# lukedan/libfluid

Hardware: AMD Instinct MI355X
Metric: particle_steps_per_sec (higher is better)
Workload: dtype f32

## Files before the change

### include/libfluid_amd.h

```cpp
#ifndef LIBFLUID_AMD_H
#define LIBFLUID_AMD_H

#include <stddef.h>
#include <stdint.h>

#ifdef __cplusplus
extern "C" {
#endif

typedef struct lfa_sim lfa_sim;

enum {
	LFA_OK = 0,
	LFA_E_INVALID = -1,
	LFA_E_NO_DEVICE = -2,
	LFA_E_HIP = -3,
	LFA_E_OOM = -4,
	LFA_E_NAN = -5,
	LFA_E_UNSUPPORTED = -6,
	LFA_W_PCG_NOT_CONVERGED = 1
};

enum { LFA_PIC = 0, LFA_FLIP_BLEND = 1, LFA_APIC = 2 };
enum { LFA_P2G_LDS_BINNED = 0, LFA_P2G_GLOBAL_ATOMIC = 1 };
// ... 115 lines not shown
int lfa_mesher_create_window(lfa_mesher **out, const uint64_t size[3], const double grid_offset[3], double cell_size,
                             double particle_extent, uint64_t cell_radius, uint64_t zlo, uint64_t zhi, int device);
int lfa_mesher_window(const lfa_mesher *m, uint64_t *z0, uint64_t *n_planes, uint64_t *own_lo, uint64_t *own_hi);
int lfa_mesher_sample_ids(lfa_mesher *m, const double *positions, const uint32_t *ids, uint64_t n, double r);
int lfa_mesher_rebase(lfa_mesher *m, uint64_t vertices_below);
int lfa_mesher_create(lfa_mesher **out, const uint64_t size[3], const double grid_offset[3], double cell_size,
                      double particle_extent, uint64_t cell_radius, int device);
void lfa_mesher_destroy(lfa_mesher *m);
const char *lfa_mesher_last_error(const lfa_mesher *m);
int lfa_mesher_sample(lfa_mesher *m, const double *positions, uint64_t n, double r);
int lfa_mesher_sample_sim(lfa_mesher *m, lfa_sim *s, double r);
int lfa_mesher_download_values(lfa_mesher *m, double *values);
int lfa_mesher_upload_values(lfa_mesher *m, const double *values);
int lfa_mesher_marching_cubes(lfa_mesher *m, uint64_t *n_vertices, uint64_t *n_indices);
int lfa_mesher_download_mesh(lfa_mesher *m, double *positions, uint64_t *indices);
int lfa_mesher_normals(lfa_mesher *m);
int lfa_mesher_download_normals(lfa_mesher *m, double *normals);
int lfa_mesher_normals_time(lfa_mesher *m, double *ms);
int lfa_mesher_boundary_size(lfa_mesher *m, uint64_t *n_cells, uint64_t *n_triangles);
int lfa_mesher_download_boundary(lfa_mesher *m, uint8_t *cases, double *face);
int lfa_mesher_window_normals(lfa_mesher *m, const uint8_t *cases_above, const double *face_above, uint64_t n_triangles_above);
int lfa_mesher_window_normals_from(lfa_mesher *m, lfa_mesher *above);

#define LFA_NUM_TIMERS 10
int lfa_enable_timing(lfa_sim *s, int on);
int lfa_get_timings(lfa_sim *s, double ms[LFA_NUM_TIMERS]);
int lfa_get_counts(lfa_sim *s, uint64_t counts[5]);
#define LFA_NUM_SOLVER_STATS 8
int lfa_get_solver_stats(lfa_sim *s, uint64_t stats[LFA_NUM_SOLVER_STATS]);
#define LFA_MAX_MG_LEVELS 12
int lfa_get_mg_level_tiles(lfa_sim *s, uint64_t tiles[LFA_MAX_MG_LEVELS]);
int lfa_get_correction_stats(lfa_sim *s, uint64_t stats[2]);
int lfa_get_correction_stats_ex(lfa_sim *s, uint64_t stats[3]);

enum {
	LFA_K_SPMV_DOT = 0,
	LFA_K_AXPY_MAX = 1,
	LFA_K_MIC_APPLY = 2,
	LFA_K_UPDATE_S = 3,
	LFA_K_P2G_SCATTER = 4,
	LFA_K_P2G_FINALIZE = 5,
	LFA_K_G2P = 6,
	LFA_K_BIN = 7,
	LFA_K_MIC_FINE = 8,
	LFA_K_COARSE = 9,
	LFA_K_PCG_A = 10,
	LFA_K_PCG_B = 11,
	LFA_K_MG_AXPY_PRESMOOTH = 12,
	LFA_K_MG_DOWN0 = 13,
	LFA_K_MG_COARSE = 14,
	LFA_K_MG_UP0 = 15
};
int lfa_bench_kernel(lfa_sim *s, int which, int reps, double *mean_ms);
int lfa_bench_stream(lfa_sim *s, uint64_t bytes, int reps, double *copy_gbs, double *read_gbs);
void lfa_pool_trim(void);
void lfa_pool_stats(uint64_t stats[4]);
const char *lfa_bench_stream_variant(void);

#ifdef __cplusplus
}
#endif
#endif
```

### libfluid_amd/__init__.py

```python
import ctypes as C
import os

import numpy as np

from . import scenes
from .scenes import CELL_DTYPE, PARTICLE_DTYPE

HERE = os.path.dirname(os.path.abspath(__file__))
LIB_PATH = os.path.join(HERE, "libfluid_amd.so")

PIC, FLIP_BLEND, APIC = 0, 1, 2
P2G_LDS_BINNED, P2G_GLOBAL_ATOMIC = 0, 1
PRECOND_MIC0_TILED, PRECOND_MIC0_EXACT, PRECOND_MULTILEVEL, PRECOND_MULTIGRID = 0, 1, 2, 3
PCG_F32, PCG_F64 = 0, 1
OK, W_PCG_NOT_CONVERGED = 0, 1
NUM_TIMERS = 10
NUM_STEP_TIMERS = 16
STEP_TIMER_NAMES = ["advect_collide", "bin", "p2g", "p2g_scatter_kernel", "build_system", "pcg_loop", "apply_pressure",
                    "correct_cell_index", "correct_tiled_kernel", "correct_collide", "extrapolate", "g2p", "time_step",
                    "pcg_iterations", "pcg_iteration_mean", "overlapped"]
TIMER_NAMES = ["bin", "p2g", "gravity", "build_system", "pcg_loop", "apply_pressure", "extrapolate", "g2p",
               "p2g_scatter_kernel", "pcg_iteration_mean"]


# ... 95 lines not shown
    "lfa_mesher_create": (_int, [C.POINTER(_vp), _vp, _vp, _dbl, _dbl, _u64, _int]),
    "lfa_mesher_create_window": (_int, [C.POINTER(_vp), _vp, _vp, _dbl, _dbl, _u64, _u64, _u64, _int]),
    "lfa_mesher_window": (_int, [_vp, C.POINTER(_u64), C.POINTER(_u64), C.POINTER(_u64), C.POINTER(_u64)]),
    "lfa_mesher_sample_ids": (_int, [_vp, _vp, _vp, _u64, _dbl]),
    "lfa_mesher_rebase": (_int, [_vp, _u64]),
    "lfa_mesher_destroy": (None, [_vp]),
    "lfa_mesher_last_error": (C.c_char_p, [_vp]),
    "lfa_mesher_sample": (_int, [_vp, _vp, _u64, _dbl]),
    "lfa_mesher_sample_sim": (_int, [_vp, _vp, _dbl]),
    "lfa_mesher_download_values": (_int, [_vp, _vp]),
    "lfa_mesher_upload_values": (_int, [_vp, _vp]),
    "lfa_mesher_marching_cubes": (_int, [_vp, C.POINTER(_u64), C.POINTER(_u64)]),
    "lfa_mesher_download_mesh": (_int, [_vp, _vp, _vp]),
    "lfa_mesher_normals": (_int, [_vp]),
    "lfa_mesher_download_normals": (_int, [_vp, _vp]),
    "lfa_mesher_normals_time": (_int, [_vp, C.POINTER(_dbl)]),
    "lfa_mesher_boundary_size": (_int, [_vp, C.POINTER(_u64), C.POINTER(_u64)]),
    "lfa_mesher_download_boundary": (_int, [_vp, _vp, _vp]),
    "lfa_mesher_window_normals": (_int, [_vp, _vp, _vp, _u64]),
    "lfa_mesher_window_normals_from": (_int, [_vp, _vp]),
    "lfa_clear_sources": (_int, [_vp]),
    "lfa_add_source": (_int, [_vp, _vp, _u64, _vp, _u64, _int, _int]),
    "lfa_update_sources": (_int, [_vp, C.POINTER(_u64)]),
    "lfa_advect_collide": (_int, [_vp, _dbl]),
    "lfa_advect": (_int, [_vp, _dbl]),
    "lfa_correct": (_int, [_vp, _dbl]),
    "lfa_collide": (_int, [_vp]),
    "lfa_correct_collide": (_int, [_vp, _dbl]),
    "lfa_time_step": (_int, [_vp, _dbl, C.POINTER(_dbl), C.POINTER(_u64)]),
    "lfa_get_step_timings": (_int, [_vp, C.POINTER(_dbl * NUM_STEP_TIMERS)]),
    "lfa_set_step_overlap": (_int, [_vp, _int]),
    "lfa_get_correction_stats": (_int, [_vp, C.POINTER(_u64 * 2)]),
    "lfa_get_correction_stats_ex": (_int, [_vp, C.POINTER(_u64 * 3)]),
    "lfa_correct_collide_begin": (_int, [_vp, _dbl]),
    "lfa_correct_collide_end": (_int, [_vp]),
    "lfa_correct_collide_undo": (_int, [_vp]),
    "lfa_dist_unique_id": (_int, [_vp]),
    "lfa_dist_init_rccl": (_int, [_vp, _int, _int, _vp, _vp]),
    "lfa_dist_local_hub_create": (_vp, [_int]),
    "lfa_dist_local_hub_destroy": (None, [_vp]),
    "lfa_dist_init_local": (_int, [_vp, _vp, _int, _vp]),
    "lfa_dist_init_shm": (_int, [_vp, C.c_char_p, _int, _int, _vp]),
    "lfa_dist_get_slab": (_int, [_vp, C.POINTER(C.c_int32), C.POINTER(C.c_int32)]),
    "lfa_dist_abandon": (_int, [_vp]),
}
KERNELS = {"spmv_dot": 0, "axpy_max": 1, "mic_apply_dot": 2, "update_s": 3, "p2g_scatter": 4, "p2g_finalize": 5,
           "g2p": 6, "bin": 7, "mic_fine": 8, "coarse_levels": 9, "pcg_a": 10, "pcg_b": 11,
           "mg_axpy_presmooth": 12, "mg_down0": 13, "mg_coarse": 14, "mg_up0": 15}


def load_library():
    global _lib
    if _lib is None:
        path = os.environ.get("LFA_LIB_PATH") or LIB_PATH
        if not os.path.exists(path):
            raise ImportError(
                f"{path} is missing: build it with `python -c 'import __graft_entry__ as g; g.build()'` "
                "(there is no CPU fallback for the hot path)")
        lib = C.CDLL(path)
        for name, (res, args) in SIGNATURES.items():
            fn = getattr(lib, name)
            fn.restype, fn.argtypes = res, args
        _lib = lib
    return _lib


# ... 488 lines not shown

    def correct_collide(self, dt):
        self._chk(self.lib.lfa_correct_collide(self.h, float(dt)))

    def correct_collide_begin(self, dt):
        self._chk(self.lib.lfa_correct_collide_begin(self.h, float(dt)))

    def correct_collide_end(self):
        self._chk(self.lib.lfa_correct_collide_end(self.h))

    def correct_collide_undo(self):
        self._chk(self.lib.lfa_correct_collide_undo(self.h))

    def time_step(self, dt):
        res, it = C.c_double(0.0), C.c_uint64(0)
        rc = self._chk(self.lib.lfa_time_step(self.h, float(dt), C.byref(res), C.byref(it)))
        return res.value, it.value, rc

    def step_timings(self):
        arr = (C.c_double * NUM_STEP_TIMERS)()
        self._chk(self.lib.lfa_get_step_timings(self.h, C.byref(arr)))
        return dict(zip(STEP_TIMER_NAMES, list(arr)))

    def correction_stats(self):
        arr = (C.c_uint64 * 2)()
        self._chk(self.lib.lfa_get_correction_stats(self.h, C.byref(arr)))
        return int(arr[0]), int(arr[1])

    def correction_stats_ex(self):
        arr = (C.c_uint64 * 3)()
        self._chk(self.lib.lfa_get_correction_stats_ex(self.h, C.byref(arr)))
        return int(arr[0]), int(arr[1]), int(arr[2])

    def set_step_overlap(self, on):
        self._chk(self.lib.lfa_set_step_overlap(self.h, int(bool(on))))

    def init_local_slab(self, hub, rank, layer_bounds):
        b = np.ascontiguousarray(layer_bounds, dtype=np.int32)
        self._chk(self.lib.lfa_dist_init_local(self.h, hub, int(rank), _ptr(b)))

    def init_rccl_slab(self, rank, nranks, unique_id, layer_bounds):
        b = np.ascontiguousarray(layer_bounds, dtype=np.int32)
        uid = np.frombuffer(bytes(unique_id), dtype=np.uint8).copy()
        self._chk(self.lib.lfa_dist_init_rccl(self.h, int(rank), int(nranks), _ptr(uid), _ptr(b)))

    def init_shm_slab(self, name, rank, nranks, layer_bounds):
        b = np.ascontiguousarray(layer_bounds, dtype=np.int32)
        self._chk(self.lib.lfa_dist_init_shm(self.h, str(name).encode(), int(rank), int(nranks), _ptr(b)))

    def abandon_transport(self):
        self._chk(self.lib.lfa_dist_abandon(self.h))

    def slab(self):
        lo, hi = C.c_int32(0), C.c_int32(0)
        self._chk(self.lib.lfa_dist_get_slab(self.h, C.byref(lo), C.byref(hi)))
        return lo.value, hi.value

    def enable_timing(self, on=True):
        self._chk(self.lib.lfa_enable_timing(self.h, 1 if on else 0))

    def timings(self):
        arr = (C.c_double * NUM_TIMERS)()
        self._chk(self.lib.lfa_get_timings(self.h, C.byref(arr)))
        return dict(zip(TIMER_NAMES, list(arr)))

    def bench_kernel(self, name, reps=20):
# ... 29 lines not shown
```

### libfluid_amd/csrc/particles.hip

```cpp
#include <math.h>

#include <algorithm>
#include <utility>

#include "common.h"
#include "pcg.h"

namespace {

__device__ inline bool solid_or_outside(const GridDims &g, const uint8_t *solid, int x, int y, int z) {
	if (!in_grid(g, x, y, z)) return true;
	return solid[blocked_index(g, x, y, z)] != 0;
}

__device__ inline void collide(const GridDims &g, const uint8_t *solid, double from[3], double to[3], double skin) {
	for (int bounce = 0; bounce < 3; ++bounce) {
		bool hit = false;
		double diff[3], inv[3], t[3];
		int cur[3], last[3], adv[3];
#pragma unroll
		for (int d = 0; d < 3; ++d) {
			cur[d] = (int)floor(from[d]);
			last[d] = (int)floor(to[d]);
			diff[d] = to[d] - from[d];
// ... 58 lines not shown
		const double cp = to[d] - (double)ci;
		double x = to[d];
		if (cp < skin && ci == 0) x += skin - cp;
		if (cp > skin_max && ci + 1 >= n[d]) x += skin_max - cp;
		to[d] = x;
	}
}

__device__ inline void cell_of_key(const GridDims &g, uint32_t key, int c[3]) {
	int tile = (int)(key >> 9), l = (int)(key & 511), tx, ty, tz;
	tile_coords(g, tile, tx, ty, tz);
	c[0] = tx * 8 + (l & 7); c[1] = ty * 8 + ((l >> 3) & 7); c[2] = tz * 8 + (l >> 6);
}
__device__ inline void split_position(double p, int n, int &cell, float &t) {
	double m = p < 0.0 ? 0.0 : p;
	int c = m >= (double)n ? n - 1 : (int)m;
	double td = p - (double)c;
	float tf = (float)td;
	if (!(tf > 0.0f)) tf = 0.0f;
	if (td < 1.0 && tf >= 1.0f) tf = 0.99999994f;
	if (tf > 1.0f) tf = 1.0f;
	cell = c;
	t = tf;
}

#ifndef CORR_PARTS
#define CORR_PARTS 2
#endif
#define CORR_THREADS 512
#define CORR_THREADS_BIG 1024
#ifndef CORR_STAGE_DEPTH
#define CORR_STAGE_DEPTH 4
#endif
#define CORR_BIG_SLICES 4

struct MoveParams {
	double dt_over_h;
	double skin;
	double corr;
	double inv_re2;
	float *c_home;
	size_t c_home_stride;
	int collide;
};

__global__ void __launch_bounds__(256) k_tile_has_solid(const uint8_t *solid, int nt, uint8_t *tile_solid) {
	for (int t = blockIdx.x; t < nt; t += gridDim.x) {
		const uint8_t *c = solid + (size_t)t * LFA_TILE_CELLS;
		const int any = __syncthreads_or((c[threadIdx.x] | c[threadIdx.x + 256]) != 0);
		if (threadIdx.x == 0) tile_solid[t] = (uint8_t)(any ? 1 : 0);
	}
}
__global__ void k_tile_clear(GridDims g, const uint8_t *tile_solid, uint8_t *tile_clear) {
	const int t = blockIdx.x * blockDim.x + threadIdx.x;
	if (t >= g.nt) return;
	int tx, ty, tz;
	tile_coords(g, t, tx, ty, tz);
	int any = 0;
	for (int dz = -1; dz <= 1; ++dz)
		for (int dy = -1; dy <= 1; ++dy)
			for (int dx = -1; dx <= 1; ++dx) {
				const int x = tx + dx, y = ty + dy, z = tz + dz;
				if ((unsigned)x < (unsigned)g.ntx && (unsigned)y < (unsigned)g.nty && (unsigned)z < (unsigned)g.ntz)
					any |= tile_solid[x + g.ntx * (y + g.nty * z)];
			}
	tile_clear[t] = (uint8_t)(any ? 0 : 1);
// ... 57 lines not shown
}

#define AC_CHUNKS 8
template <bool COERCE>
__global__ void __launch_bounds__(256)
k_advect_collide_count(size_t n, ParticleSoA p, GridDims g, const uint8_t *solid, MoveParams mp, const uint8_t *coerce_map,
                       const float *src_vel, const uint8_t *tile_clear, uint32_t *tile_count, uint32_t *rank) {
	const int lane = threadIdx.x & 63;
	const size_t wave = ((size_t)blockIdx.x * blockDim.x + threadIdx.x) >> 6;
	const size_t i0 = wave * (64 * AC_CHUNKS) + lane;
	uint32_t tile[AC_CHUNKS], my_rank[AC_CHUNKS];
#pragma unroll
	for (int c = 0; c < AC_CHUNKS; ++c) {
		const size_t i = i0 + 64 * c;
		const uint32_t k = i < n ? advect_one<COERCE>(i, p, g, solid, mp, coerce_map, src_vel, tile_clear) : 0xFFFFFFFFu;
		tile[c] = k != 0xFFFFFFFFu ? k >> 9 : 0xFFFFFFFFu;
	}
	lfa_wave_tile_ranks(tile, tile_count, my_rank);
#pragma unroll
	for (int c = 0; c < AC_CHUNKS; ++c) {
		const size_t i = i0 + 64 * c;
		if (tile[c] != 0xFFFFFFFFu) rank[i] = my_rank[c];
	}
}

__device__ inline float hash_unit(uint32_t a, uint32_t b, uint32_t k) {
	uint32_t x = a * 0x9E3779B1u ^ (b + 0x7F4A7C15u) * 0x85EBCA77u ^ k * 0xC2B2AE3Du;
	x ^= x >> 15; x *= 0x2C1B3C6Du; x ^= x >> 12; x *= 0x297A2D39u; x ^= x >> 15;
	return (float)(x >> 8) * (2.0f / 16777216.0f) - 1.0f;
}

#define FT 11
#define FT3 (FT * FT * FT)
#define FT_STRIDE (FT3 + 1)
#define FT_INV 1.375f
#define FT_PL ((FT + CORR_PARTS - 1) / CORR_PARTS)
#define FB 13
#define FBZ (FT_PL + 2)
#define FB_N (FB * FB * FBZ)
#define FB_ROWS (FB * FBZ)
#define FINE_CAP 5632
#define FINE_CAP_BIG 12288
#define FIDX_THREADS 512
#define FIDX_CNT 1536
#define FIDX_STAGE 4608

__device__ inline int fine_coord(int l, float t) {
	const int f = (int)(((float)l + t) * FT_INV);
	return f < FT - 1 ? f : FT - 1;
}
__device__ inline float4 fine_record(int lx, int ly, int lz, float t0, float t1, float t2, uint32_t index) {
	const uint32_t b0 = (__float_as_uint(t0) & 0x3FFFFFFFu) | ((uint32_t)(lx & 3) << 30);
	const uint32_t b1 = (__float_as_uint(t1) & 0x3FFFFFFFu) | ((uint32_t)(lx >> 2) << 31) | ((uint32_t)(ly & 1) << 30);
	const uint32_t b2 = (__float_as_uint(t2) & 0x3FFFFFFFu) | ((uint32_t)(lz & 1) << 31);
	return make_float4(__uint_as_float(b0), __uint_as_float(b1), __uint_as_float(b2), __uint_as_float(index));
}
__device__ inline void fine_decode(const float4 &r, int fy, int fz, float t[3], int l[3]) {
	const uint32_t b0 = __float_as_uint(r.x), b1 = __float_as_uint(r.y), b2 = __float_as_uint(r.z);
	t[0] = __uint_as_float(b0 & 0x3FFFFFFFu); t[1] = __uint_as_float(b1 & 0x3FFFFFFFu); t[2] = __uint_as_float(b2 & 0x3FFFFFFFu);
	l[0] = (int)(b0 >> 30) | ((int)(b1 >> 31) << 2);
	const int y0 = (8 * fy) / FT, z0 = (8 * fz) / FT;
	l[1] = y0 + ((y0 ^ (int)(b1 >> 30)) & 1);
	l[2] = z0 + ((z0 ^ (int)(b2 >> 31)) & 1);
}

__global__ void __launch_bounds__(FIDX_THREADS)
k_build_fine_index(const int *ptiles, int n_ptiles, const uint32_t *key, const float *t0, const float *t1, const float *t2,
                   const uint32_t *tile_start, const uint32_t *tile_count, uint32_t *fine_start, float4 *spos, uint32_t *key_copy) {
	__shared__ uint32_t cnt[FIDX_CNT];
	__shared__ uint32_t wsum[FIDX_THREADS / 64];
	__shared__ float4 stage[FIDX_STAGE];
	static_assert(FIDX_CNT % FIDX_THREADS == 0 && FIDX_STAGE % FIDX_THREADS == 0, "index kernel sizing");
	constexpr int PER = FIDX_CNT / FIDX_THREADS;
	auto fine_of = [&](uint32_t i, int l[3], float t[3]) -> int {
		const uint32_t k = key[i];
		l[0] = (int)(k & 7); l[1] = (int)((k >> 3) & 7); l[2] = (int)((k >> 6) & 7);
		t[0] = t0[i]; t[1] = t1[i]; t[2] = t2[i];
		return fine_coord(l[0], t[0]) + FT * (fine_coord(l[1], t[1]) + FT * fine_coord(l[2], t[2]));
	};
	constexpr int RPT = FIDX_STAGE / FIDX_THREADS;
	for (int slot = blockIdx.x; slot < n_ptiles; slot += gridDim.x) {
		const int tile = ptiles[slot];
		const uint32_t b = tile_start[tile], e = b + tile_count[tile];
		const bool staged = e - b <= FIDX_STAGE;
#pragma unroll
		for (int k = 0; k < PER; ++k) cnt[threadIdx.x + FIDX_THREADS * k] = 0;
		__syncthreads();
		uint32_t rf[RPT];
		float r0[RPT], r1[RPT], r2[RPT];
		if (staged) {
#pragma unroll
			for (int r = 0; r < RPT; ++r) {
				const uint32_t i = b + threadIdx.x + FIDX_THREADS * r;
				rf[r] = 0xFFFFFFFFu;
				if (i < e) {
					int l[3];
					float t[3];
					const int f = fine_of(i, l, t);
					rf[r] = ((uint32_t)f << 9) | (uint32_t)(l[0] | (l[1] << 3) | (l[2] << 6));
					r0[r] = t[0]; r1[r] = t[1]; r2[r] = t[2];
					atomicAdd(&cnt[f], 1u);
				}
			}
		} else {
			for (uint32_t i = b + threadIdx.x; i < e; i += FIDX_THREADS) {
				int l[3];
				float t[3];
				atomicAdd(&cnt[fine_of(i, l, t)], 1u);
			}
		}
		__syncthreads();
		uint32_t c[PER], incl = 0;
#pragma unroll
		for (int k = 0; k < PER; ++k) {
			c[k] = cnt[PER * threadIdx.x + k];
			incl += c[k];
		}
		const uint32_t sum = incl;
		const int lane = threadIdx.x & 63, wid = threadIdx.x >> 6;
#pragma unroll
		for (int o = 1; o < 64; o <<= 1) {
			uint32_t t = __shfl_up(incl, o, 64);
			if (lane >= o) incl += t;
		}
		if (lane == 63) wsum[wid] = incl;
		__syncthreads();
		uint32_t ex = b + incl - sum;
		for (int w = 0; w < wid; ++w) ex += wsum[w];
		__syncthreads();
#pragma unroll
		for (int k = 0; k < PER; ++k) {
			const int f = PER * threadIdx.x + k;
			cnt[f] = ex;
			if (f <= FT3) fine_start[(size_t)tile * FT_STRIDE + f] = ex;
			ex += c[k];
		}
		__syncthreads();
		if (staged) {
#pragma unroll
			for (int r = 0; r < RPT; ++r)
				if (rf[r] != 0xFFFFFFFFu) {
					const uint32_t at = atomicAdd(&cnt[rf[r] >> 9], 1u);
					stage[at - b] = fine_record((int)(rf[r] & 7), (int)((rf[r] >> 3) & 7), (int)((rf[r] >> 6) & 7), r0[r], r1[r], r2[r],
					                            b + threadIdx.x + FIDX_THREADS * r);
				}
			if (key_copy) {
#pragma unroll
				for (int r = 0; r < RPT; ++r)
					if (rf[r] != 0xFFFFFFFFu) key_copy[b + threadIdx.x + FIDX_THREADS * r] = ((uint32_t)tile << 9) | (rf[r] & 511u);
			}
			__syncthreads();
			for (uint32_t k = threadIdx.x; k < e - b; k += FIDX_THREADS) spos[b + k] = stage[k];
		} else {
			for (uint32_t i = b + threadIdx.x; i < e; i += FIDX_THREADS) {
				int l[3];
				float t[3];
				const uint32_t at = atomicAdd(&cnt[fine_of(i, l, t)], 1u);
				spos[at] = fine_record(l[0], l[1], l[2], t[0], t[1], t[2], i);
				if (key_copy) key_copy[i] = key[i];
			}
		}
		__syncthreads();
	}
}

__device__ inline int fine_source(const GridDims &g, const uint32_t *tile_count, int tx, int ty, int tz, int gx, int gy, int gz, int &fx,
                                  int &fy, int &fz) {
	const int dx = gx < 0 ? -1 : (gx >= FT ? 1 : 0), dy = gy < 0 ? -1 : (gy >= FT ? 1 : 0), dz = gz < 0 ? -1 : (gz >= FT ? 1 : 0);
	fx = gx - FT * dx; fy = gy - FT * dy; fz = gz - FT * dz;
	const int x = tx + dx, y = ty + dy, z = tz + dz;
	if ((unsigned)x >= (unsigned)g.ntx || (unsigned)y >= (unsigned)g.nty || (unsigned)z >= (unsigned)g.ntz) return -1;
	const int tile = x + g.ntx * (y + g.nty * z);
	return tile_count[tile] ? tile : -1;
}

__device__ inline void correct_collide_record(size_t rk, const ParticleSoA &p, uint32_t *out_key, float *out_tx, float *out_ty, float *out_tz,
                                              const GridDims &g, const uint8_t *solid, const uint32_t *tile_count, const uint32_t *fine_start,
                                              const float4 *spos, const MoveParams &mp, const uint32_t *only_flagged, const int *tile_pslot,
                                              int p_off, const uint32_t *key_before) {
	const float4 me = spos[rk];
	const size_t i = __float_as_uint(me.w);
	const uint32_t key_i = key_before ? key_before[i] : p.key[i];
	if (key_i == 0xFFFFFFFFu) return;
	const int tile = (int)(key_i >> 9);
	const int l[3] = {(int)(key_i & 7), (int)((key_i >> 3) & 7), (int)((key_i >> 6) & 7)};
	const float t[3] = {__uint_as_float(__float_as_uint(me.x) & 0x3FFFFFFFu), __uint_as_float(__float_as_uint(me.y) & 0x3FFFFFFFu),
// ... 63 lines not shown
                   const uint8_t *solid, const uint32_t *tile_count, const uint32_t *fine_start, const float4 *spos, MoveParams mp,
                   const uint32_t *only_flagged, const int *tile_pslot, int p_off, const uint32_t *key_before) {
	if (only_flagged && only_flagged[0] == 0) return;
	for (size_t rk = (size_t)blockIdx.x * blockDim.x + threadIdx.x; rk < n; rk += (size_t)gridDim.x * blockDim.x)
		correct_collide_record(rk, p, out_key, out_tx, out_ty, out_tz, g, solid, tile_count, fine_start, spos, mp, only_flagged, tile_pslot,
		                       p_off, key_before);
}

#ifdef CORR_PROFILE
__device__ unsigned long long g_corr_prof[8];
#define CORR_STAMP(k)                                                                   \
	do {                                                                                \
		if (!ONLY && threadIdx.x == 0) {                                                \
			const unsigned long long now_ = wall_clock64();                             \
			atomicAdd(&g_corr_prof[k], now_ - stamp_);                                  \
			stamp_ = now_;                                                              \
		}                                                                               \
	} while (0)
#else
#define CORR_STAMP(k) do { } while (0)
#endif
template <int CAP, bool ONLY>
__global__ void __launch_bounds__(ONLY ? CORR_THREADS_BIG : CORR_THREADS, 4)
k_correct_fine(const int *ptiles, int n_ptiles, uint32_t *out_key, float *out_tx, float *out_ty, float *out_tz, GridDims g,
                const uint8_t *solid, const uint32_t *tile_count, const uint32_t *fine_start, const float4 *spos, MoveParams mp,
                uint32_t *overflow_tiles, const uint8_t *tile_clear, const uint32_t *only) {
	constexpr int T = ONLY ? CORR_THREADS_BIG : CORR_THREADS;
	constexpr int CNT = ((FB_N + 1 + T - 1) / T) * T;
	__shared__ float px[CAP], py[CAP], pz[CAP];
	__shared__ uint32_t fcnt[CNT];
	__shared__ uint16_t foff[FB_N + 1];
	__shared__ uint32_t rowsrc[FB_ROWS * 3];
	__shared__ uint32_t ownoff[FT * FT_PL + 1];
	__shared__ int srct[27];
	__shared__ uint32_t wsum[T / 64];
	uint16_t *own = (uint16_t *)fcnt;
	static_assert(CNT > FB_N && CNT % T == 0, "fcnt sizing");
	constexpr int PER = CNT / T;
	const int nn[3] = {g.nx, g.ny, g.nz};
	const int lane = threadIdx.x & 63, wid = threadIdx.x >> 6;
	if (ONLY && only[0] == 0) return;
	constexpr int SLICES = ONLY ? CORR_BIG_SLICES : 1;
	for (int item = blockIdx.x; item < SLICES * CORR_PARTS * n_ptiles; item += gridDim.x) {
		const int work = item / SLICES, slice = item % SLICES;
		if (ONLY && !((only[1 + (work >> 5)] >> (work & 31)) & 1u)) continue;
		const int tile = ptiles[work / CORR_PARTS], part = work % CORR_PARTS;
		int tx, ty, tz;
		tile_coords(g, tile, tx, ty, tz);
		const int own_lo = part * FT_PL, own_n = (own_lo + FT_PL <= FT ? FT_PL : FT - own_lo);
		const int gz0 = own_lo - 1;
		const int nzb = own_n + 2;
		const int nrows = FB * nzb, nown_rows = FT * (nzb - 2);
		const bool open_water = (tile_clear[tile] & 1) != 0;
		__syncthreads();
#ifdef CORR_PROFILE
		unsigned long long stamp_ = wall_clock64();
		if (!ONLY && threadIdx.x == 0) atomicAdd(&g_corr_prof[7], 1ull);
#endif
		if (threadIdx.x < 27) {
			int fx, fy, fz;
			srct[threadIdx.x] = fine_source(g, tile_count, tx, ty, tz, FT * ((int)threadIdx.x % 3 - 1), FT * (((int)threadIdx.x / 3) % 3 - 1),
			                                FT * ((int)threadIdx.x / 9 - 1), fx, fy, fz);
		}
		__syncthreads();
#pragma unroll
		for (int k = 0; k < PER; ++k) {
			const int f = threadIdx.x + T * k;
			uint32_t cnt = 0, src0 = 0;
			if (f < FB * nrows) {
				const int bx = f % FB, row = f / FB, by = row % FB, bz = row / FB;
				const int gx = bx - 1, gy = by - 1, gz = gz0 + bz;
				const int dx = gx < 0 ? 0 : (gx >= FT ? 2 : 1), dy = gy < 0 ? 0 : (gy >= FT ? 2 : 1), dz = gz < 0 ? 0 : (gz >= FT ? 2 : 1);
				const int src = srct[dx + 3 * dy + 9 * dz];
				if (src >= 0) {
					const uint32_t fid = (uint32_t)((gx - FT * (dx - 1)) + FT * ((gy - FT * (dy - 1)) + FT * (gz - FT * (dz - 1))));
					const uint32_t *fs = fine_start + ((uint32_t)src * FT_STRIDE + fid);
					src0 = fs[0];
					cnt = fs[1] - src0;
				}
				if (bx <= 1 || bx == FB - 1) rowsrc[row * 3 + (bx <= 1 ? bx : 2)] = src0;
			}
			fcnt[f] = cnt;
		}
		__syncthreads();
		uint32_t c4[PER], sum = 0;
#pragma unroll
		for (int k = 0; k < PER; ++k) {
			c4[k] = fcnt[PER * threadIdx.x + k];
			sum += c4[k];
		}
		uint32_t incl = sum;
#pragma unroll
		for (int o = 1; o < 64; o <<= 1) {
			uint32_t t = __shfl_up(incl, o, 64);
			if (lane >= o) incl += t;
		}
		if (lane == 63) wsum[wid] = incl;
// ... 17 lines not shown
				const int f = PER * threadIdx.x + k;
				if (f <= FB_N) foff[f] = (uint16_t)ex;
				ex += c4[k];
			}
		}
		__syncthreads();
		uint32_t own_total = 0;
		{
			uint32_t len = 0;
			if (threadIdx.x < (unsigned)nown_rows) {
				const int row = (1 + threadIdx.x % FT) + FB * (1 + threadIdx.x / FT);
				len = (uint32_t)foff[row * FB + FB - 1] - (uint32_t)foff[row * FB + 1];
			}
			uint32_t in2 = len;
#pragma unroll
			for (int o = 1; o < 64; o <<= 1) {
				uint32_t t = __shfl_up(in2, o, 64);
				if (lane >= o) in2 += t;
			}
			if (lane == 63) wsum[wid] = in2;
			__syncthreads();
			uint32_t wo = 0;
			for (int w = 0; w < T / 64; ++w) {
				if (w < wid) wo += wsum[w];
				own_total += wsum[w];
			}
			if (threadIdx.x < (unsigned)nown_rows) ownoff[threadIdx.x] = wo + in2 - len;
			if (threadIdx.x == 0) ownoff[nown_rows] = own_total;
		}
		const bool listed = own_total <= 2u * CNT;
		__syncthreads();
		CORR_STAMP(0);
		{
			auto locate = [&](uint32_t slot, uint32_t &src, int &seg, int &dy, int &dz, int &fy, int &fz, int &ownslot) {
				int r = 0;
#pragma unroll
				for (int step = 64; step; step >>= 1) {
					const int c = r + step;
					if (c < nrows && (uint32_t)foff[c * FB] <= slot) r = c;
				}
				const int by = r % FB, bz = r / FB;
				const int gy = by - 1, gz = gz0 + bz;
				dy = gy < 0 ? -1 : (gy >= FT ? 1 : 0); dz = gz < 0 ? -1 : (gz >= FT ? 1 : 0);
				fy = gy - FT * dy; fz = gz - FT * dz;
				const uint32_t d0 = foff[r * FB], d1 = foff[r * FB + 1], d2 = foff[r * FB + FB - 1];
				seg = slot < d1 ? 0 : (slot < d2 ? 1 : 2);
				src = rowsrc[r * 3 + seg] + (slot - (seg == 0 ? d0 : (seg == 1 ? d1 : d2)));
				ownslot = (listed && seg == 1 && by >= 1 && by <= FT && bz >= 1 && bz <= nzb - 2)
				              ? (int)(ownoff[(by - 1) + FT * (bz - 1)] + (slot - d1)) : -1;
			};
			auto put = [&](uint32_t slot, const float4 &rec, int seg, int dy, int dz, int fy, int fz, int ownslot) {
				float t[3];
				int l[3];
				fine_decode(rec, fy, fz, t, l);
				px[slot] = (float)(8 * (seg - 1) + l[0]) + t[0];
				py[slot] = (float)(8 * dy + l[1]) + t[1];
				pz[slot] = (float)(8 * dz + l[2]) + t[2];
				if (ownslot >= 0) own[ownslot] = (uint16_t)slot;
			};
			for (uint32_t slot0 = threadIdx.x; slot0 < total; slot0 += CORR_STAGE_DEPTH * T) {
				uint32_t src[CORR_STAGE_DEPTH];
				int meta[CORR_STAGE_DEPTH], ownslot[CORR_STAGE_DEPTH];
				float4 rec[CORR_STAGE_DEPTH];
#pragma unroll
				for (int u = 0; u < CORR_STAGE_DEPTH; ++u) {
					const uint32_t slot = slot0 + u * T;
// ... 13 lines not shown
						put(slot, rec[u], meta[u] & 3, ((meta[u] >> 2) & 3) - 1, ((meta[u] >> 4) & 3) - 1, (meta[u] >> 6) & 15, (meta[u] >> 10) & 15, ownslot[u]);
				}
			}
		}
		__syncthreads();
		CORR_STAMP(1);
#ifdef CORR_PROFILE
		if (!ONLY && threadIdx.x == 0) { atomicAdd(&g_corr_prof[5], (unsigned long long)total); atomicAdd(&g_corr_prof[6], (unsigned long long)own_total); }
#endif
		for (uint32_t w = threadIdx.x + T * slice; w < own_total; w += T * SLICES) {
			uint32_t me;
			if (listed) {
				me = own[w];
			} else {
				int lo = 0, hi = nown_rows - 1;
				while (lo < hi) {
					const int mid = (lo + hi + 1) >> 1;
					if (ownoff[mid] <= w) lo = mid;
					else hi = mid - 1;
				}
				me = (uint32_t)foff[((1 + lo % FT) + FB * (1 + lo / FT)) * FB + 1] + (w - ownoff[lo]);
			}
#ifdef CORR_PROFILE
			const unsigned long long w0_ = wall_clock64();
#endif
			const float mx = px[me], my = py[me], mz = pz[me];
			int fx = (int)(mx * FT_INV), fy = (int)(my * FT_INV), fz = (int)(mz * FT_INV);
			fx = fx < FT - 1 ? fx : FT - 1; fy = fy < FT - 1 ? fy : FT - 1; fz = fz < FT - 1 ? fz : FT - 1;
			const int bx = fx + 1, by = fy + 1, bz = fz - gz0;
			float sx = 0.f, sy = 0.f, sz = 0.f;
			typedef float f2 __attribute__((ext_vector_type(2)));
			f2 s2x = 0.f, s2y = 0.f, s2z = 0.f;
			const float inv_re2 = (float)mp.inv_re2;
			uint32_t j = 0xFFFFFFFFu;
			const uint32_t myrow = by + FB * bz;
			const uint32_t grec = rowsrc[myrow * 3 + 1] + (me - (uint32_t)foff[myrow * FB + 1]);
			auto pair2 = [&](uint32_t q, f2 qx, f2 qy, f2 qz) {
				const f2 dx = mx - qx, dy = my - qy, dz = mz - qz;
				const f2 d2 = __builtin_elementwise_fma(dz, dz, __builtin_elementwise_fma(dy, dy, dx * dx));
				const f2 kl = __builtin_elementwise_fma(-d2, (f2)inv_re2, (f2)1.0f);
				if (kl.x > 0.0f || kl.y > 0.0f) {
#pragma unroll
					for (int k = 0; k < 2; ++k) {
						const float d2k = k ? d2.y : d2.x, klk = k ? kl.y : kl.x;
						if (!(klk > 0.0f)) continue;
						if (d2k < 1e-12f) {
							if (q + k != me) {
								if (j == 0xFFFFFFFFu) j = __float_as_uint(spos[grec].w);
								sx += hash_unit(j, q + k, 0); sy += hash_unit(j, q + k, 1); sz += hash_unit(j, q + k, 2);
							}
						} else {
							const float f = klk * klk * klk * rsqrtf(d2k);
							sx += f * (k ? dx.y : dx.x); sy += f * (k ? dy.y : dy.x); sz += f * (k ? dz.y : dz.x);
						}
					}
				}
			};
			auto walk = [&](auto &&p2, auto &&p2_centre) {
				for (int dz = -1; dz <= 1; ++dz)
					for (int dy = -1; dy <= 1; ++dy) {
						const int rowf = FB * ((by + dy) + FB * (bz + dz)) + bx;
						const uint32_t b = foff[rowf - 1], e = foff[rowf + 2];
						auto run = [&](auto &&pp) {
							uint32_t q = b;
							for (; q + 4 <= e; q += 4) {
								const float x0 = px[q], x1 = px[q + 1], x2 = px[q + 2], x3 = px[q + 3];
								const float y0 = py[q], y1 = py[q + 1], y2 = py[q + 2], y3 = py[q + 3];
								const float z0 = pz[q], z1 = pz[q + 1], z2 = pz[q + 2], z3 = pz[q + 3];
								pp(q, f2{x0, x1}, f2{y0, y1}, f2{z0, z1});
								pp(q + 2, f2{x2, x3}, f2{y2, y3}, f2{z2, z3});
							}
							if (q + 2 <= e) {
								pp(q, f2{px[q], px[q + 1]}, f2{py[q], py[q + 1]}, f2{pz[q], pz[q + 1]});
								q += 2;
							}
							if (q < e) pp(q, f2{px[q], 1e6f}, f2{py[q], 1e6f}, f2{pz[q], 1e6f});
						};
						if (dy == 0 && dz == 0) run(p2_centre);
						else run(p2);
					}
			};
			float d2_min = 1.0f;
			uint32_t n_tiny = 0;
			auto fast = [&](f2 qx, f2 qy, f2 qz) -> f2 {
				const f2 dx = mx - qx, dy = my - qy, dz = mz - qz;
				const f2 d2 = __builtin_elementwise_fma(dz, dz, __builtin_elementwise_fma(dy, dy, __builtin_elementwise_fma(dx, dx, (f2)1e-30f)));
				f2 kl;
				kl.x = __builtin_amdgcn_fmed3f(__builtin_fmaf(-d2.x, inv_re2, 1.0f), 0.0f, 1.0f);
				kl.y = __builtin_amdgcn_fmed3f(__builtin_fmaf(-d2.y, inv_re2, 1.0f), 0.0f, 1.0f);
				f2 f = kl * kl * kl;
				f.x *= __builtin_amdgcn_rsqf(d2.x);
				f.y *= __builtin_amdgcn_rsqf(d2.y);
				s2x = __builtin_elementwise_fma(f, dx, s2x);
				s2y = __builtin_elementwise_fma(f, dy, s2y);
				s2z = __builtin_elementwise_fma(f, dz, s2z);
				return d2;
			};
			walk([&](uint32_t, f2 qx, f2 qy, f2 qz) {
					     const f2 d2 = fast(qx, qy, qz);
					     d2_min = fminf(d2_min, fminf(d2.x, d2.y));
				     },
				     [&](uint32_t, f2 qx, f2 qy, f2 qz) {
					     const f2 d2 = fast(qx, qy, qz);
					     n_tiny += (d2.x < 1e-12f ? 1u : 0u) + (d2.y < 1e-12f ? 1u : 0u);
				     });
			if (d2_min < 1e-12f || n_tiny != 1u) {
				s2x = 0.f; s2y = 0.f; s2z = 0.f;
				walk(pair2, pair2);
			}
			sx += s2x.x + s2x.y;
			sy += s2y.x + s2y.y;
			sz += s2z.x + s2z.y;
#ifdef CORR_PROFILE
			if (!ONLY && threadIdx.x == 0) atomicAdd(&g_corr_prof[4], wall_clock64() - w0_);
#endif
			float tme[3];
			int lme[3];
			const float4 rec = spos[grec];
			fine_decode(rec, fy, fz, tme, lme);
			const uint32_t jj = __float_as_uint(rec.w);
			const int c[3] = {8 * tx + lme[0], 8 * ty + lme[1], 8 * tz + lme[2]};
			const double spring[3] = {(double)sx, (double)sy, (double)sz};
			double from[3], to[3];
#pragma unroll
			for (int d = 0; d < 3; ++d) {
				from[d] = (double)c[d] + (double)tme[d];
				double x = from[d] + spring[d] * mp.corr;
				to[d] = x < 0.0 ? 0.0 : ((double)nn[d] < x ? (double)nn[d] : x);
			}
			if (mp.collide) {
				if (!open_water || fabs(to[0] - from[0]) >= 7.0 || fabs(to[1] - from[1]) >= 7.0 || fabs(to[2] - from[2]) >= 7.0)
					collide(g, solid, from, to, mp.skin);
				else
					collide_walls_only(g, to, mp.skin);
			}
			int nc[3];
			float nt[3];
#pragma unroll
			for (int d = 0; d < 3; ++d) split_position(to[d], nn[d], nc[d], nt[d]);
			out_key[jj] = blocked_index(g, nc[0], nc[1], nc[2]);
			out_tx[jj] = nt[0]; out_ty[jj] = nt[1]; out_tz[jj] = nt[2];
// ... 629 lines not shown
	}
	if (residual) *residual = res;
	if (iterations) *iterations = it;
	return rc;
}

extern "C" int lfa_get_correction_stats(lfa_sim *s, uint64_t stats[2]) {
	if (!s || !stats) return LFA_E_INVALID;
	stats[0] = stats[1] = 0;
	uint64_t ex[3];
	LFA_TRY(lfa_get_correction_stats_ex(s, ex));
	stats[0] = ex[0];
	stats[1] = ex[1];
	return LFA_OK;
}

extern "C" int lfa_get_correction_stats_ex(lfa_sim *s, uint64_t stats[3]) {
	if (!s || !stats) return LFA_E_INVALID;
	stats[0] = stats[1] = stats[2] = 0;
	if (!s->corr_ovf) return LFA_OK;
	LFA_HIP(s, hipSetDevice(s->device));
	LFA_TRY(lfa_corr_join(s));
	const size_t ovf_stride = ((size_t)CORR_PARTS * s->g.nt + 31) / 32 + 2;
	uint32_t first = 0, second = 0;
	LFA_HIP(s, hipMemcpyAsync(&first, s->corr_ovf, 4, hipMemcpyDeviceToHost, s->stream));
	LFA_HIP(s, hipMemcpyAsync(&second, s->corr_ovf + ovf_stride, 4, hipMemcpyDeviceToHost, s->stream));
	LFA_HIP(s, hipStreamSynchronize(s->stream));
	stats[0] = second;
	stats[1] = (uint64_t)CORR_PARTS * (uint64_t)s->corr_parts_tiles;
	stats[2] = first;
	return LFA_OK;
}

extern "C" int lfa_set_step_overlap(lfa_sim *s, int on) {
	if (!s) return LFA_E_INVALID;
	s->overlap_correction = on != 0;
	return LFA_OK;
}

extern "C" int lfa_get_step_timings(lfa_sim *s, double ms[LFA_NUM_STEP_TIMERS]) {
	if (!s || !ms) return LFA_E_INVALID;
	for (int k = 0; k < LFA_NUM_STEP_TIMERS; ++k) ms[k] = s->ms_next[k];
	return LFA_OK;
}
```

Before: 4.944 billion.

## Sort fine-cell particle records by x and trim out-of-reach neighbour spans

```diff
diff --git a/include/libfluid_amd.h b/include/libfluid_amd.h
--- a/include/libfluid_amd.h
+++ b/include/libfluid_amd.h
@@ -171,6 +171,8 @@
 int lfa_get_mg_level_tiles(lfa_sim *s, uint64_t tiles[LFA_MAX_MG_LEVELS]);
 int lfa_get_correction_stats(lfa_sim *s, uint64_t stats[2]);
 int lfa_get_correction_stats_ex(lfa_sim *s, uint64_t stats[3]);
+int lfa_get_fine_records(lfa_sim *s, uint64_t layout[2], uint32_t *fine_start, uint64_t fine_words, float *records,
+                         uint64_t n_records);
 
 enum {
 	LFA_K_SPMV_DOT = 0,
diff --git a/libfluid_amd/__init__.py b/libfluid_amd/__init__.py
--- a/libfluid_amd/__init__.py
+++ b/libfluid_amd/__init__.py
@@ -151,6 +151,7 @@
     "lfa_set_step_overlap": (_int, [_vp, _int]),
     "lfa_get_correction_stats": (_int, [_vp, C.POINTER(_u64 * 2)]),
     "lfa_get_correction_stats_ex": (_int, [_vp, C.POINTER(_u64 * 3)]),
+    "lfa_get_fine_records": (_int, [_vp, C.POINTER(_u64 * 2), _vp, _u64, _vp, _u64]),
     "lfa_correct_collide_begin": (_int, [_vp, _dbl]),
     "lfa_correct_collide_end": (_int, [_vp]),
     "lfa_correct_collide_undo": (_int, [_vp]),
@@ -705,6 +706,17 @@
         self._chk(self.lib.lfa_get_correction_stats_ex(self.h, C.byref(arr)))
         return int(arr[0]), int(arr[1]), int(arr[2])
 
+    def fine_records(self):
+        layout = (C.c_uint64 * 2)()
+        self._chk(self.lib.lfa_get_fine_records(self.h, C.byref(layout), None, 0, None, 0))
+        stride, nt = int(layout[0]), int(layout[1])
+        n = self.counts()["particles"]
+        fine = np.zeros((nt, stride), np.uint32)
+        rec = np.zeros((n, 4), np.uint32)
+        self._chk(self.lib.lfa_get_fine_records(self.h, C.byref(layout), fine.ctypes.data_as(C.c_void_p), fine.size,
+                                                rec.ctypes.data_as(C.c_void_p), n))
+        return fine, rec
+
     def set_step_overlap(self, on):
         self._chk(self.lib.lfa_set_step_overlap(self.h, int(bool(on))))
 
diff --git a/libfluid_amd/csrc/particles.hip b/libfluid_amd/csrc/particles.hip
--- a/libfluid_amd/csrc/particles.hip
+++ b/libfluid_amd/csrc/particles.hip
@@ -114,6 +114,15 @@
 #ifndef CORR_STAGE_DEPTH
 #define CORR_STAGE_DEPTH 4
 #endif
+#ifndef CORR_TRIM_K
+#define CORR_TRIM_K 4
+#endif
+#ifndef CORR_TRIM_LOOP
+#define CORR_TRIM_LOOP 1
+#endif
+#ifndef CORR_TRIM_LINEAR
+#define CORR_TRIM_LINEAR 0
+#endif
 #define CORR_BIG_SLICES 4
 
 struct MoveParams {
@@ -237,7 +246,8 @@
 
 #define FT 11
 #define FT3 (FT * FT * FT)
-#define FT_STRIDE (FT3 + 1)
+#define FT_STRIDE (FT3 + 2)
+#define FT_XSORTED (FT3 + 1)
 #define FT_INV 1.375f
 #define FT_PL ((FT + CORR_PARTS - 1) / CORR_PARTS)
 #define FB 13
@@ -249,6 +259,8 @@
 #define FIDX_THREADS 512
 #define FIDX_CNT 1536
 #define FIDX_STAGE 4608
+#define FIDX_SORT_SMALL 24
+#define FIDX_SORT_BIG 64
 
 __device__ inline int fine_coord(int l, float t) {
 	const int f = (int)(((float)l + t) * FT_INV);
@@ -269,12 +281,19 @@
 	l[2] = z0 + ((z0 ^ (int)(b2 >> 31)) & 1);
 }
 
+__device__ inline uint64_t fine_xkey(const float4 &r) {
+	const uint32_t b0 = __float_as_uint(r.x), b1 = __float_as_uint(r.y);
+	return ((uint64_t)(b1 >> 31) << 32) | b0;
+}
+
 __global__ void __launch_bounds__(FIDX_THREADS)
 k_build_fine_index(const int *ptiles, int n_ptiles, const uint32_t *key, const float *t0, const float *t1, const float *t2,
                    const uint32_t *tile_start, const uint32_t *tile_count, uint32_t *fine_start, float4 *spos, uint32_t *key_copy) {
 	__shared__ uint32_t cnt[FIDX_CNT];
 	__shared__ uint32_t wsum[FIDX_THREADS / 64];
 	__shared__ float4 stage[FIDX_STAGE];
+	__shared__ uint16_t big[FIDX_SORT_BIG];
+	__shared__ uint32_t nbig;
 	static_assert(FIDX_CNT % FIDX_THREADS == 0 && FIDX_STAGE % FIDX_THREADS == 0, "index kernel sizing");
 	constexpr int PER = FIDX_CNT / FIDX_THREADS;
 	auto fine_of = [&](uint32_t i, int l[3], float t[3]) -> int {
@@ -290,6 +309,7 @@
 		const bool staged = e - b <= FIDX_STAGE;
 #pragma unroll
 		for (int k = 0; k < PER; ++k) cnt[threadIdx.x + FIDX_THREADS * k] = 0;
+		if (threadIdx.x == 0) nbig = 0;
 		__syncthreads();
 		uint32_t rf[RPT];
 		float r0[RPT], r1[RPT], r2[RPT];
@@ -355,8 +375,58 @@
 					if (rf[r] != 0xFFFFFFFFu) key_copy[b + threadIdx.x + FIDX_THREADS * r] = ((uint32_t)tile << 9) | (rf[r] & 511u);
 			}
 			__syncthreads();
+			for (int f = threadIdx.x; f < FT3; f += FIDX_THREADS) {
+				const uint32_t s0 = (f ? cnt[f - 1] : b) - b, s1 = cnt[f] - b;
+				if (s1 - s0 > FIDX_SORT_SMALL) {
+					const uint32_t at = atomicAdd(&nbig, 1u);
+					if (at < FIDX_SORT_BIG) big[at] = (uint16_t)f;
+					continue;
+				}
+				for (uint32_t i = s0 + 1; i < s1; ++i) {
+					const float4 r = stage[i];
+					const uint64_t kr = fine_xkey(r);
+					uint32_t j = i;
+					for (; j > s0; --j) {
+						const float4 o = stage[j - 1];
+						if (fine_xkey(o) <= kr) break;
+						stage[j] = o;
+					}
+					if (j != i) stage[j] = r;
+				}
+			}
+			__syncthreads();
+			const bool sorted = nbig <= FIDX_SORT_BIG;
+			const uint32_t n_big = sorted ? nbig : 0u;
+			for (uint32_t w = 0; w < n_big; ++w) {
+				const int f = big[w];
+				const uint32_t s0 = (f ? cnt[f - 1] : b) - b, s1 = cnt[f] - b;
+				float4 r[RPT];
+				uint32_t rank[RPT];
+#pragma unroll
+				for (int u = 0; u < RPT; ++u) {
+					const uint32_t i = s0 + threadIdx.x + FIDX_THREADS * u;
+					rank[u] = 0xFFFFFFFFu;
+					if (i < s1) {
+						r[u] = stage[i];
+						const uint64_t kr = fine_xkey(r[u]);
+						uint32_t before = 0;
+						for (uint32_t k = s0; k < s1; ++k) {
+							const uint64_t ko = fine_xkey(stage[k]);
+							before += (ko < kr || (ko == kr && k < i)) ? 1u : 0u;
+						}
+						rank[u] = s0 + before;
+					}
+				}
+				__syncthreads();
+#pragma unroll
+				for (int u = 0; u < RPT; ++u)
+					if (rank[u] != 0xFFFFFFFFu) stage[rank[u]] = r[u];
+				__syncthreads();
+			}
+			if (threadIdx.x == 0) fine_start[(size_t)tile * FT_STRIDE + FT_XSORTED] = sorted ? 1u : 0u;
 			for (uint32_t k = threadIdx.x; k < e - b; k += FIDX_THREADS) spos[b + k] = stage[k];
 		} else {
+			if (threadIdx.x == 0) fine_start[(size_t)tile * FT_STRIDE + FT_XSORTED] = 0u;
 			for (uint32_t i = b + threadIdx.x; i < e; i += FIDX_THREADS) {
 				int l[3];
 				float t[3];
@@ -486,7 +556,7 @@
 	__shared__ uint16_t foff[FB_N + 1];
 	__shared__ uint32_t rowsrc[FB_ROWS * 3];
 	__shared__ uint32_t ownoff[FT * FT_PL + 1];
-	__shared__ int srct[27];
+	__shared__ int srct[28];
 	__shared__ uint32_t wsum[T / 64];
 	uint16_t *own = (uint16_t *)fcnt;
 	static_assert(CNT > FB_N && CNT % T == 0, "fcnt sizing");
@@ -494,6 +564,7 @@
 	const int nn[3] = {g.nx, g.ny, g.nz};
 	const int lane = threadIdx.x & 63, wid = threadIdx.x >> 6;
 	if (ONLY && only[0] == 0) return;
+	const float reach = (float)(sqrt(1.0 / mp.inv_re2) * (1.0 + 1e-6) + 1e-6);
 	constexpr int SLICES = ONLY ? CORR_BIG_SLICES : 1;
 	for (int item = blockIdx.x; item < SLICES * CORR_PARTS * n_ptiles; item += gridDim.x) {
 		const int work = item / SLICES, slice = item % SLICES;
@@ -511,12 +582,26 @@
 		unsigned long long stamp_ = wall_clock64();
 		if (!ONLY && threadIdx.x == 0) atomicAdd(&g_corr_prof[7], 1ull);
 #endif
-		if (threadIdx.x < 27) {
-			int fx, fy, fz;
-			srct[threadIdx.x] = fine_source(g, tile_count, tx, ty, tz, FT * ((int)threadIdx.x % 3 - 1), FT * (((int)threadIdx.x / 3) % 3 - 1),
-			                                FT * ((int)threadIdx.x / 9 - 1), fx, fy, fz);
+		if (wid == 0) {
+			bool unsorted = false;
+			if (threadIdx.x < 27) {
+				const int x = tx + (int)threadIdx.x % 3 - 1, y = ty + ((int)threadIdx.x / 3) % 3 - 1, z = tz + (int)threadIdx.x / 9 - 1;
+				int src = -1;
+				if ((unsigned)x < (unsigned)g.ntx && (unsigned)y < (unsigned)g.nty && (unsigned)z < (unsigned)g.ntz) {
+					const int nb = x + g.ntx * (y + g.nty * z);
+					const uint32_t have = tile_count[nb], xs = fine_start[(uint32_t)nb * FT_STRIDE + FT_XSORTED];
+					if (have) {
+						src = nb;
+						unsorted = xs == 0u;
+					}
+				}
+				srct[threadIdx.x] = src;
+			}
+			const unsigned long long any_unsorted = __ballot(unsorted);
+			if (lane == 0) srct[27] = any_unsorted == 0ull;
 		}
 		__syncthreads();
+		const bool xsorted = __builtin_amdgcn_readfirstlane(srct[27]) != 0;
 #pragma unroll
 		for (int k = 0; k < PER; ++k) {
 			const int f = threadIdx.x + T * k;
@@ -600,6 +685,7 @@
 		__syncthreads();
 		CORR_STAMP(0);
 		{
+			static_assert(FB_ROWS <= 127, "the row search below takes seven steps from 64: rows 0 .. 127");
 			auto locate = [&](uint32_t slot, uint32_t &src, int &seg, int &dy, int &dz, int &fy, int &fz, int &ownslot) {
 				int r = 0;
 #pragma unroll
@@ -679,6 +765,7 @@
 			typedef float f2 __attribute__((ext_vector_type(2)));
 			f2 s2x = 0.f, s2y = 0.f, s2z = 0.f;
 			const float inv_re2 = (float)mp.inv_re2;
+			const float x_lo = mx - reach, x_hi = mx + reach;
 			uint32_t j = 0xFFFFFFFFu;
 			const uint32_t myrow = by + FB * bz;
 			const uint32_t grec = rowsrc[myrow * 3 + 1] + (me - (uint32_t)foff[myrow * FB + 1]);
@@ -703,11 +790,32 @@
 					}
 				}
 			};
-			auto walk = [&](auto &&p2, auto &&p2_centre) {
+			auto walk = [&](auto &&p2, auto &&p2_centre, bool trim) {
 				for (int dz = -1; dz <= 1; ++dz)
 					for (int dy = -1; dy <= 1; ++dy) {
 						const int rowf = FB * ((by + dy) + FB * (bz + dz)) + bx;
-						const uint32_t b = foff[rowf - 1], e = foff[rowf + 2];
+						uint32_t b = foff[rowf - 1], e = foff[rowf + 2];
+						if (trim) {
+#if CORR_TRIM_LINEAR
+							while (b < e && fmaf(-((mx - px[b]) * (mx - px[b])), inv_re2, 1.0f) <= 0.0f) ++b;
+							while (b < e && fmaf(-((mx - px[e - 1]) * (mx - px[e - 1])), inv_re2, 1.0f) <= 0.0f) --e;
+#else
+							for (;;) {
+								if (e - b < (uint32_t)CORR_TRIM_K) break;
+								uint32_t nl = 0, nr = 0;
+								bool goon_l = true, goon_r = true;
+#pragma unroll
+								for (int k = 0; k < CORR_TRIM_K; ++k) {
+									goon_l = goon_l && px[b + k] < x_lo;
+									goon_r = goon_r && px[e - 1 - k] > x_hi;
+									nl += goon_l ? 1u : 0u;
+									nr += goon_r ? 1u : 0u;
+								}
+								b += nl; e -= nr;
+								if (!CORR_TRIM_LOOP || (!goon_l && !goon_r)) break;
+							}
+#endif
+						}
 						auto run = [&](auto &&pp) {
 							uint32_t q = b;
 							for (; q + 4 <= e; q += 4) {
@@ -750,10 +858,10 @@
 				     [&](uint32_t, f2 qx, f2 qy, f2 qz) {
 					     const f2 d2 = fast(qx, qy, qz);
 					     n_tiny += (d2.x < 1e-12f ? 1u : 0u) + (d2.y < 1e-12f ? 1u : 0u);
-				     });
+				     }, xsorted);
 			if (d2_min < 1e-12f || n_tiny != 1u) {
 				s2x = 0.f; s2y = 0.f; s2z = 0.f;
-				walk(pair2, pair2);
+				walk(pair2, pair2, false);
 			}
 			sx += s2x.x + s2x.y;
 			sy += s2y.x + s2y.y;
@@ -1449,6 +1557,21 @@
 	return LFA_OK;
 }
 
+extern "C" int lfa_get_fine_records(lfa_sim *s, uint64_t layout[2], uint32_t *fine_start, uint64_t fine_words, float *records,
+                                    uint64_t n_records) {
+	if (!s || !layout) return LFA_E_INVALID;
+	layout[0] = FT_STRIDE;
+	layout[1] = (uint64_t)s->g.nt;
+	if (!s->fine_start) return (fine_start && fine_words) || (records && n_records) ? LFA_E_INVALID : LFA_OK;
+	if (fine_words > (uint64_t)s->g.nt * FT_STRIDE || n_records > s->np_live) return LFA_E_INVALID;
+	LFA_HIP(s, hipSetDevice(s->device));
+	LFA_TRY(lfa_corr_join(s));
+	if (fine_start && fine_words) LFA_HIP(s, hipMemcpyAsync(fine_start, s->fine_start, fine_words * 4, hipMemcpyDeviceToHost, s->stream));
+	if (records && n_records) LFA_HIP(s, hipMemcpyAsync(records, correction_scratch(s), n_records * 16, hipMemcpyDeviceToHost, s->stream));
+	LFA_HIP(s, hipStreamSynchronize(s->stream));
+	return LFA_OK;
+}
+
 extern "C" int lfa_set_step_overlap(lfa_sim *s, int on) {
 	if (!s) return LFA_E_INVALID;
 	s->overlap_correction = on != 0;
```

Result: slower. 4.502 billion (-8.9%).
